# micropilot/myosuite-mjx

Hardware: AMD Instinct MI355X
Metric: env-steps/s (whole node) myoHandPoseRandom-v0 batch 4096 (higher is better)
Workload: dtype f32

## Files before the change

### myosuite_mjx_amd/csrc/myo_host.h

```cpp
#ifndef MYO_HOST_H
#define MYO_HOST_H

#include <memory>

static int g_lanes = 64;
static thread_local std::string g_err;
static int fail(int code, const std::string& msg) { g_err = msg; return code; }
#define HIPCHK(x) do { hipError_t e_ = (x); if (e_ != hipSuccess) return fail(MYO_E_HIP, std::string(#x) + ": " + hipGetErrorString(e_)); } while (0)

struct DevPool {
  std::vector<void*> ptrs;
  DevPool() = default;
  DevPool(const DevPool&) = delete;
  DevPool& operator=(const DevPool&) = delete;
  ~DevPool() { for (void* p : ptrs) (void)hipFree(p); }
  template <class T> int alloc(T** out, size_t nbytes, bool zero = true) {
    void* p = nullptr;
    const hipError_t e = hipMalloc(&p, nbytes);
    if (e != hipSuccess) return fail(e == hipErrorOutOfMemory ? MYO_E_NOMEM : MYO_E_HIP, std::string("hipMalloc: ") + hipGetErrorString(e));
    ptrs.push_back(p);
    if (zero) HIPCHK(hipMemset(p, 0, nbytes));
    *out = (T*)p;
    return MYO_OK;
  }
// ... 101 lines not shown
  bool obj_ok = false;
  std::vector<int> geom_type0, geom_body0, geom_priority0;
  std::vector<double> geom_size0, geom_pos0, geom_friction0, body_mass_d;
};

struct myo_episode { float *run = nullptr, *last = nullptr; uint8_t* finished = nullptr; int* count = nullptr; };

struct myo_obs_terms { float *terms = nullptr, *sel = nullptr, *prop = nullptr; const int2* prog = nullptr; const float* cst = nullptr; int wt = 0, ws = 0, wp = 0; };

struct myo_batch {
  const myo_model* model = nullptr;
  DevBatch db{};
  TaskDev task{};
  int ntarget_alloc = 0, obs_alloc = 0, env_offset = 0;
  DevPool pool;
  float *d_tlo = nullptr, *d_thi = nullptr, *d_init = nullptr, *d_jlo = nullptr, *d_jhi = nullptr, *d_action = nullptr, *d_rnd = nullptr;
  float* d_initv = nullptr;
  float *d_init2 = nullptr, *d_initv2 = nullptr, *d_fatvec = nullptr;
  const char* last_kernel = "step_kernel";
  DevWalk* d_walk = nullptr;
  DevTrack* d_track = nullptr;
  float* d_metrics = nullptr;
  int track_frames = 0;
  int track_flavour = 0;
  ResetArgs *d_reset = nullptr, reset_args{};
  uint64_t reset_seed = 0;
  hipEvent_t ev0 = nullptr, ev1 = nullptr;
  uint64_t bench_step = 0;
  long long* d_stamps = nullptr;
  int* d_order = nullptr;
  int* d_sched = nullptr;
  int sched_stride = 0;
  int balance = 1;
  bool bm_on = false;
  bool bp_on = false;
  int bq_body = -1;
  bool sens_on = false;
  myo_episode episode;
  myo_obs_terms obs_terms;
  bool bq_on = false;
  bool fwd_on = false;
  void* fwd_buf[16] = {};
  bool obj_on = false;
  std::vector<int> obj_geoms, obj_bodies;
  float *d_objk = nullptr, *d_obj_draw = nullptr;
  int* d_obj_draw_k = nullptr;
  std::vector<hipEvent_t> kev;
  int kev_pending = 0;
  float last_kernel_ms = 0.f;
  ~myo_batch() {
    for (hipEvent_t e : kev) (void)hipEventDestroy(e);
    if (ev0) (void)hipEventDestroy(ev0);
    if (ev1) (void)hipEventDestroy(ev1);
  }
};

struct DevBuf { void* p; size_t width, elem; };
typedef int (*BufFamily)(const myo_batch*, int which, DevBuf*);
static int buf_out(const DevBuf& d, void** dev_ptr, size_t* pitch, size_t* width) { *dev_ptr = d.p; *pitch = *width = d.width; return MYO_OK; }
static int copy_blocking(int device, void* dst, const void* src, size_t nbytes, hipMemcpyKind kind) {
  HIPCHK(hipSetDevice(device));
  HIPCHK(hipDeviceSynchronize());
  if (nbytes) HIPCHK(hipMemcpy(dst, src, nbytes, kind));
  return MYO_OK;
}
static int copy_to_host(int device, void* host, const void* dev, size_t nbytes) { return copy_blocking(device, host, dev, nbytes, hipMemcpyDeviceToHost); }
// ... 15 lines not shown

struct RwdCols { const char* const* name; int n; };
struct ObsDims { int nq, nv, nu, na, ntip, pose_act; };
enum { OBS_SRC_ROW = 0,
       OBS_SRC_TIME = 1,
       OBS_SRC_TARGET = 2,
       OBS_SRC_QPOS = 3,
       OBS_SRC_ACT = 4,
       OBS_SRC_CONST = 5 };
struct ObsTerm { const char* name; int width, src, idx; };
struct ObsTable : std::vector<ObsTerm> { int dim = 0; };

struct TaskHooks {
  int (*configure)(myo_batch*, const myo_task_config*);
  int (*obs)(myo_batch*, hipStream_t, int obs_only, int reset_only);
  int (*post)(myo_batch*, hipStream_t, uint64_t seed, int auto_max);
  RwdCols rwd;
  void (*obs_terms)(const ObsDims&, ObsTable&);
};
static const TaskHooks* task_hooks(int task);
static int launch_step(myo_batch* b, const float* action, int actmap, int nsub, hipStream_t s, int kflags = 0);

template <class Task> static int launch_task_obs(myo_batch* b, hipStream_t s, int obs_only, int reset_only) {
  hipLaunchKernelGGL(task_obs_kernel<Task>, dim3(b->db.B), dim3(64), 0, s, b->model->dm, b->db, b->task, (const DevTrack*)b->d_track, b->reset_seed, obs_only, reset_only);
  return MYO_OK;
}
static int sync_reset_args(myo_batch* b, hipStream_t s) {
  if (!b->d_reset) { const int rc = b->pool.alloc(&b->d_reset, sizeof(ResetArgs), false); if (rc) return rc; }
  else if (!memcmp(&b->reset_args.Bt, &b->db, sizeof(DevBatch)) && !memcmp(&b->reset_args.T, &b->task, sizeof(TaskDev))) return MYO_OK;
  memcpy(&b->reset_args.Bt, &b->db, sizeof(DevBatch)); memcpy(&b->reset_args.T, &b->task, sizeof(TaskDev));
  HIPCHK(hipMemcpyAsync(b->d_reset, &b->reset_args, sizeof(ResetArgs), hipMemcpyHostToDevice, s));
  return MYO_OK;
}
template <class Task> static int launch_task_post(myo_batch* b, hipStream_t s, uint64_t seed, int auto_max) {
  const int rc = sync_reset_args(b, s);
  if (rc) return rc;
  hipLaunchKernelGGL(task_post_kernel<Task>, dim3(b->db.B), dim3(64), 0, s, b->model->dm, b->db, b->task, (const DevTrack*)b->d_track,
                     (const ResetArgs*)b->d_reset, b->model->nq, b->model->dm.qpos0, seed, b->env_offset, auto_max);
  return MYO_OK;
}

static int root_link_of_dofs(const myo_model* m, int d0, int n) {
  const int l = m->dof_link[d0];
  if (m->link_parent[l] >= 0 || m->link_dofnum[l] != n) return -1;
  for (int k = 1; k < n; k++) if (m->dof_link[d0 + k] != l) return -1;
  return l;
}

static void quat2mat_d(double* R, const double* q) {
  const double w = q[0], x = q[1], y = q[2], z = q[3];
  R[0] = w * w + x * x - y * y - z * z; R[1] = 2 * (x * y - w * z); R[2] = 2 * (x * z + w * y);
  R[3] = 2 * (x * y + w * z); R[4] = w * w - x * x + y * y - z * z; R[5] = 2 * (y * z - w * x);
  R[6] = 2 * (x * z - w * y); R[7] = 2 * (y * z + w * x); R[8] = w * w - x * x - y * y + z * z;
}

#endif
```

### myosuite_mjx_amd/csrc/myo_host_batch.h

```cpp
#ifndef MYO_HOST_BATCH_H
#define MYO_HOST_BATCH_H

static int batch_create(const myo_model* m, int B, myo_batch** out) {
  HIPCHK(hipSetDevice(m->device));
  std::unique_ptr<myo_batch> owner(new myo_batch());
  myo_batch* b = owner.get();
  DevBatch& d = b->db;
  int nv = m->dm.nv, nu = m->dm.nu, nq = m->nq, rc;
  b->model = m; d.B = B; b->ntarget_alloc = nv > 24 ? nv : 24; b->obs_alloc = 3 * nv + 4 * nu + 64;
  b->sched_stride = (B + 7) / 8 + 1;
  if (m->wave_ok) {
    const int kc = m->wave_cfg == 0 ? 8 : 20, nj = m->trk ? 4 : 3;
    d.ovf_row = 8 + nj * kc + (kc + 3) / 4 + (m->trk ? TRK_STATE : 0);
    d.ovf_rows = m->trk ? NCX2 : NCX;
  }
#define BA(ptr, n) if ((rc = b->pool.alloc(&ptr, (size_t)(n) * 4))) return rc;
  BA(d.qpos, (size_t)B * nq) BA(d.qvel, (size_t)B * nv) BA(d.act, (size_t)B * nu) BA(d.ctrl, (size_t)B * nu) BA(d.warm, (size_t)B * nv)
  BA(d.time, B) BA(d.target, (size_t)B * b->ntarget_alloc) BA(d.obs, (size_t)B * b->obs_alloc) BA(d.reward, B) BA(d.done, B)
  BA(d.solved, B) BA(d.qacc, (size_t)B * nv) BA(d.tenlen, (size_t)B * nu) BA(d.actforce, (size_t)B * nu) BA(d.sitexpos, (size_t)B * 24)
  BA(d.flags, B) BA(d.diag, (size_t)B * 8) BA(d.elapsed, B) BA(d.episode, B) BA(d.mprw, (size_t)B * 64)
  BA(b->d_tlo, b->ntarget_alloc) BA(b->d_thi, b->ntarget_alloc) BA(b->d_init, nq) BA(b->d_jlo, nv) BA(b->d_jhi, nv) BA(b->d_rnd, 4 * (size_t)nq)
  BA(b->d_action, (size_t)B * nu) BA(d.fatigue, (size_t)B * 3 * nu)
  if (m->trk) { BA(d.linkx, (size_t)B * 12 * m->dm.nl) }
  if (m->wave_ok) { BA(d.ovf, (size_t)B * d.ovf_rows * d.ovf_row) BA(d.ovf_cand, (size_t)B * NCANDX) }
// ... 227 lines not shown
  FIELD(MYO_F_ACTION, b->d_action, b->model->dm.nu),
  FIELD(MYO_F_FATIGUE, b->db.fatigue, 3 * b->model->dm.nu),
  FIELD(MYO_F_HFIELD, b->db.hfield, b->model->dw.hf.nrow * b->model->dw.hf.ncol, nullptr, "MYO_F_HFIELD: the model has no colliding height field"),
  FIELD(MYO_F_GEOMSIZE, b->db.gsize, 4, nullptr, "MYO_F_GEOMSIZE: no geom override set (myo_batch_set_geom_override)"),
  FIELD(MYO_F_LINKX, b->db.linkx, 12 * b->model->dm.nl, nullptr, "MYO_F_LINKX: this model's kernel does not export link frames"),
  FIELD(MYO_F_METRICS, b->d_metrics, 4, nullptr, "MYO_F_METRICS: the track task is not configured (myo_batch_configure_track)"),
  FIELD(MYO_F_BODYMASS, b->db.bmass, b->model->body_mass0.size(), nullptr, nullptr, &bm_override),
  FIELD(MYO_F_BODYMASS_RANGE, b->db.bmass_range, 2 * b->model->body_mass0.size(), nullptr, nullptr, &bm_override),
  FIELD(MYO_F_BODYPOS, b->db.bpos, 3, nullptr, nullptr, &bp_override),
  FIELD(MYO_F_BODYPOS_RANGE, b->db.bpos_range, 6, nullptr, nullptr, &bp_override),
  FIELD(MYO_F_BODYQUAT, b->db.bquat, 4, nullptr, nullptr, &bq_override),
  FIELD(MYO_F_BODYQUAT_RANGE, b->db.bquat_range, 6, nullptr, nullptr, &bq_override),
  FIELD(MYO_F_SENSORDATA, b->db.sens, b->db.ntouch, SENS_READ_ONLY, SENS_ABSENT),
  FIELD(MYO_F_CFRC, b->db.cfrc, 3 * (b->db.ntouch + 1), SENS_READ_ONLY, SENS_ABSENT),
};
#undef FIELD
constexpr int N_FIELDS = sizeof field_rows / sizeof field_rows[0];
constexpr bool field_rows_in_id_order(int i = 0) { return i == N_FIELDS || (field_rows[i].id == i && field_rows_in_id_order(i + 1)); }
static_assert(N_FIELDS == MYO_F_CFRC + 1 && field_rows_in_id_order(), "field_rows: one row per field id of include/myo_hip.h, in id order");

static const FieldRow* field_row(int f) { return f >= 0 && f < N_FIELDS ? &field_rows[f] : nullptr; }
static int field_info(const myo_batch* b, const FieldRow* row, DevBuf* d) {
  if (!row) return fail(MYO_E_ARG, "unknown field");
  void* p = row->ptr(b);
  if (!p && row->absent) return fail(MYO_E_ARG, row->absent);
  *d = {p, row->width(b), 4};
  return MYO_OK;
}

static int batch_field(myo_batch* b, int field, void** dev_ptr, size_t* pitch, size_t* width) {
  const FieldRow* row = field_row(field);
  DevBuf d; int rc;
  if ((row && row->ov && (rc = override_start(b, *row->ov))) || (rc = field_info(b, row, &d))) return rc;
  return buf_out(d, dev_ptr, pitch, width);
}
static int batch_read(myo_batch* b, int field, void* host, size_t nbytes) {
  const FieldRow* row = field_row(field);
  DevBuf d; int rc;
  if ((rc = field_info(b, row, &d)) || (rc = buf_check(b, d, host, nbytes, "myo_batch_read: size mismatch"))) return rc;
  if (row->ov && !(b->*row->ov->on)) return row->ov->fill_default(b, field, (float*)host, b->db.B, d.width);
  return copy_to_host(b->model->device, host, d.p, nbytes);
}
static int batch_write(myo_batch* b, int field, const void* host, size_t nbytes) {
  const FieldRow* row = field_row(field);
  DevBuf d; int rc;
  if (row && row->read_only) return fail(MYO_E_ARG, row->read_only);
  if ((rc = field_info(b, row, &d)) || (rc = buf_check(b, d, host, nbytes, "myo_batch_write: size mismatch"))) return rc;
  if (row->ov && ((rc = row->ov->validate(b, field, (const float*)host, b->db.B, d.width)) || (rc = override_start(b, *row->ov)) || (rc = field_info(b, row, &d)))) return rc;
  return copy_to_device(b->model->device, d.p, host, nbytes);
}

#endif
```

### myosuite_mjx_amd/csrc/myo_host_step.h

```cpp
#ifndef MYO_HOST_STEP_H
#define MYO_HOST_STEP_H

#define MYO_WAVE_KERNELS(X)                                                                                             \
  X(WK_HAND, "step_kernel_w<24,8,32,1,3,false,0,false>", 24, 8, 32, 1, 3, false, 0)                                      \
  X(WK_HAND_SPEC, "step_kernel_w<24,8,32,1,4,false,1,false>", 24, 8, 32, 1, 4, false, 1)                                 \
  X(WK_LEG, "step_kernel_w<36,20,32,2,2,false,0,false>", 36, 20, 32, 2, 2, false, 0)                                     \
  X(WK_LEG_SCHED, "step_kernel_w<36,20,32,2,2,true,0,false>", 36, 20, 32, 2, 2, true, 0)                                 \
  X(WK_LEG_SPEC_SCHED, "step_kernel_w<36,20,32,2,2,true,2,false>", 36, 20, 32, 2, 2, true, 2)                            \
  X(WK_LEG_SPEC, "step_kernel_w<36,20,32,2,2,false,2,false>", 36, 20, 32, 2, 2, false, 2)                                \
  X(WK_TERRAIN, "step_kernel_w<36,20,32,2,2,false,0,true>", 36, 20, 32, 2, 2, false, 0, true)                            \
  X(WK_TERRAIN_SPEC_SCHED, "step_kernel_w<36,20,32,2,2,true,3,true>", 36, 20, 32, 2, 2, true, 3, true)                   \
  X(WK_TERRAIN_SPEC, "step_kernel_w<36,20,32,2,2,false,3,true>", 36, 20, 32, 2, 2, false, 3, true)                       \
  X(WK_TRK, "step_kernel_w<36,20,32,2,2,false,0,false,true>", 36, 20, 32, 2, 2, false, 0, false, true)                   \
  X(WK_HAND_RK4, "step_kernel_w<24,8,32,1,3,false,0,false,false,true>", 24, 8, 32, 1, 3, false, 0, false, false, true)   \
  X(WK_LEG_RK4, "step_kernel_w<36,20,32,2,2,false,0,false,false,true>", 36, 20, 32, 2, 2, false, 0, false, false, true)
struct WaveKernel {
  const char* name;
  void (*fn)(const DevModel*, const DevModelW*, DevBatch, const float*, int, int, long long*, const int*, const DevWalk*, int, SchedDev);
};
enum WaveKernelId {
#define X(id, name, ...) id,
  MYO_WAVE_KERNELS(X)
#undef X
  WK_TRK_OBJ
// ... 14 lines not shown
  if (m->dw.hf.on) return m->terrain_sizes ? WK_TERRAIN_SPEC : WK_TERRAIN;
  return leg_sizes ? WK_LEG_SPEC : WK_LEG;
}

static int launch_reset(myo_batch* b, const uint8_t* mask_dev, uint64_t seed, void* stream, int max_episode_steps) {
  b->reset_seed = seed;
  const DevModel& dm = b->model->dm;
  HIPCHK(hipSetDevice(b->model->device));
  hipLaunchKernelGGL(reset_kernel, dim3(b->db.B), dim3(64), 0, (hipStream_t)stream, b->db, b->task, b->model->nq, dm.nv, dm.nu, dm.qpos0, mask_dev, seed,
                     b->env_offset, max_episode_steps);
  HIPCHK(hipGetLastError());
  return MYO_OK;
}

struct SchedPlan { bool on; int grid; SchedDev S; };
static SchedPlan sched_plan(const myo_batch* b, int nsub, bool walk, int kflags) {
  const myo_model* m = b->model;
  const int Bn = b->db.B, nsubtot = nsub + (walk ? 1 : 0);
  static const int sched_mode = [] { const char* e = getenv("MYO_SCHED"); return e ? atoi(e) : -1; }();
  const int n_cu = m->n_cu > 0 ? m->n_cu : 256;
  const int resident = n_cu * (m->wave_cfg == 0 ? 16 : (m->wave_cfg == 1 ? 8 : std::max(1, (160 * 1024) / std::max(1, m->env_lds_bytes_w))));
  const bool sched_ok = !kflags && Bn >= 64 && Bn <= SCHED_ENV_MASK && nsubtot <= 15 && nsub > 0;
  const bool on = sched_ok && !b->bm_on && m->wave_cfg == 1 && !m->rk4 && !(m->dw.hf.on && !m->terrain_sizes) && (sched_mode == 1 || (sched_mode == -1 && Bn >= 2 * resident));
  const int nqueue = std::max(1, std::min(8, n_cu / 32));
  SchedPlan P{on, Bn, SchedDev{b->d_sched, b->d_sched + 32, nqueue == 8 ? b->sched_stride : (Bn + nqueue - 1) / nqueue + 1, nsubtot, nqueue}};
  if (on) {
    P.grid = Bn < resident ? Bn : resident;
    static const int grid_override = [] { const char* e = getenv("MYO_SCHED_GRID"); return e ? atoi(e) : 0; }();
    if (grid_override > 0 && grid_override < P.grid) P.grid = grid_override;
  }
  return P;
}

static int launch_wave(myo_batch* b, const float* action, int actmap, int nsub, hipStream_t s, int kflags, const DevWalk* wk) {
  const myo_model* m = b->model;
  static OncePerDevice attr;
  int rc = set_lds_limit(attr, wave_kernels, 64 * 1024, m->device);
  if (rc) return rc;
  const int Bn = b->db.B;
  const SchedPlan P = sched_plan(b, nsub, wk != nullptr, kflags);
  const int* order = nullptr;
  if (b->balance && Bn >= 1024 && Bn % 4 == 0 && !kflags && !P.on) {
    static const int prio_mode = [] { const char* e = getenv("MYO_PRIO"); return e ? atoi(e) : 2; }();
    hipLaunchKernelGGL(balance_kernel, dim3(1), dim3(1024), 0, s, (const int*)b->db.diag, Bn, b->d_order, Bn / 4, prio_mode);
    order = b->d_order;
  }
  const WaveKernel& k = wave_kernels[select_wave_kernel(m, b->bm_on, P.on, b->obj_on)];
  if (!kflags) b->last_kernel = k.name;
  if (P.on) hipLaunchKernelGGL(sched_init_kernel, dim3(1), dim3(1024), 0, s, (const int*)b->db.diag, Bn, P.S);
  hipLaunchKernelGGL(k.fn, dim3(P.grid), dim3(64), (size_t)m->env_lds_bytes_w, s, (const DevModel*)m->d_dm, (const DevModelW*)m->d_dw, b->db, action, actmap,
                     nsub, b->d_stamps, order, wk, kflags, P.S);
  HIPCHK(hipGetLastError());
  if (wk && b->db.rwd && !(kflags & KF_OBS_ONLY)) { if ((rc = walk_terms_launch(b, s))) return rc; }
  if (wk && b->obs_terms.terms) return obs_terms_launch(b, s);
  return MYO_OK;
}

static int launch_lanes(myo_batch* b, int G, const float* action, int actmap, int nsub, hipStream_t s) {
  const myo_model* m = b->model;
  const int EPW = 64 / G, grid = (b->db.B + EPW - 1) / EPW;
  const size_t lds = (size_t)EPW * m->env_lds_bytes;
  if (G == 16) hipLaunchKernelGGL(step_kernel<16>, dim3(grid), dim3(64), lds, s, m->dm, b->db, action, actmap, nsub, b->d_stamps);
  else if (G == 32) hipLaunchKernelGGL(step_kernel<32>, dim3(grid), dim3(64), lds, s, m->dm, b->db, action, actmap, nsub, b->d_stamps);
  else hipLaunchKernelGGL(step_kernel<64>, dim3(grid), dim3(64), lds, s, m->dm, b->db, action, actmap, nsub, b->d_stamps);
  HIPCHK(hipGetLastError());
  return MYO_OK;
}

static int launch_step(myo_batch* b, const float* action, int actmap, int nsub, hipStream_t s, int kflags) {
  const myo_model* m = b->model;
  const DevWalk* wk = b->task.task == MYO_TASK_WALK ? b->d_walk : nullptr;
  if (kflags && !(wk && g_lanes == 64)) return fail(MYO_E_ARG, "observation pass: walk task on the wave kernel only");
  const int G = (g_lanes == 64 && !m->wave_ok) ? 16 : ((g_lanes != 64 && !m->generic_ok) ? 64 : g_lanes);
  const bool wave = G == 64 && m->wave_ok;
  static OncePerDevice attr;
  static const struct { const void* fn; } lanes_kernels[] = {{(const void*)step_kernel<16>}, {(const void*)step_kernel<32>}, {(const void*)step_kernel<64>}, {(const void*)reach_obs_kernel<16>}};
  int rc = set_lds_limit(attr, lanes_kernels, 160 * 1024, m->device);
  if (rc) return rc;
#if MYO_POISON
  {
    static const int pmode = [] { const char* e = getenv("MYO_POISON_MODE"); return e ? atoi(e) : 7; }();
    if (pmode & 1) hipLaunchKernelGGL(scratch_poison_kernel, dim3(16384), dim3(64), 0, s, (float*)b->d_stamps, 0);
    if (pmode & 2) hipLaunchKernelGGL(vgpr_poison_kernel, dim3(8192), dim3(64), 0, s, 0x7fc0dead);
    if (pmode & 4) hipLaunchKernelGGL(sgpr_poison_kernel, dim3(32768), dim3(64), 0, s);
  }
#endif
  if (!wave && !m->generic_ok)
    return fail(MYO_E_UNSUPPORTED, "this model (tendon limits / free joint / equalities / plane contacts) needs the wave-per-env kernel (lanes = 64)");
  if (b->sens_on && (rc = sens_check(b))) return rc;
  if (b->bm_on) {
    if ((rc = bm_check(b))) return rc;
    const int n = b->db.B * m->dm.nl;
    hipLaunchKernelGGL(link_compose_kernel, dim3((n + 255) / 256), dim3(256), 0, s, b->db, m->dm.nl, m->d_lm_adr, m->d_lm_body, m->d_lm_tab);
  }
  if ((rc = obj_compose(b, s))) return rc;
  return wave ? launch_wave(b, action, actmap, nsub, s, kflags, wk) : launch_lanes(b, G, action, actmap, nsub, s);
}

static int sum_kernel_ms(myo_batch* b, int n) {
  float tot = 0.f;
  for (int i = 0; i < n; i++) { float t; HIPCHK(hipEventElapsedTime(&t, b->kev[2 * i], b->kev[2 * i + 1])); tot += t; }
  b->last_kernel_ms = tot;
  return MYO_OK;
}

int myo_bench_rollout(myo_batch* b, int steps, int nsubsteps, uint64_t seed, int mode, int max_episode_steps, void* stream, float* ms_out) {
  if (!b || steps <= 0) return fail(MYO_E_ARG, "myo_bench_rollout: bad arguments");
  HIPCHK(hipSetDevice(b->model->device));
  hipStream_t s = (hipStream_t)stream;
  int rc;
  if (!(mode & MYO_BENCH_FRESH_ACTIONS)) { rc = myo_random_action(b, b->d_action, seed, b->bench_step, b->env_offset, stream); if (rc) return rc; }
  const int base = ms_out ? 0 : b->kev_pending;
  while ((int)b->kev.size() < 2 * (base + steps)) { hipEvent_t e; HIPCHK(hipEventCreate(&e)); b->kev.push_back(e); }
  if (ms_out) { b->kev_pending = 0; HIPCHK(hipEventRecord(b->ev0, s)); }
  for (int i = 0; i < steps; i++) {
    if (mode & MYO_BENCH_FRESH_ACTIONS) { rc = myo_random_action(b, b->d_action, seed, b->bench_step++, b->env_offset, stream); if (rc) return rc; }
    HIPCHK(hipEventRecord(b->kev[2 * (base + i)], s));
    const bool mjx_track = b->task.task == MYO_TASK_TRACK && b->track_flavour == 0;
    rc = launch_step(b, b->d_action, mjx_track ? MYO_ACTMAP_CTRLRANGE : MYO_ACTMAP_MUSCLE_SIGMOID, nsubsteps, s);
    if (rc) return rc;
    HIPCHK(hipEventRecord(b->kev[2 * (base + i) + 1], s));
    const TaskHooks* hooks = task_hooks(b->task.task);
    if (mjx_track) continue;
    if ((mode & MYO_BENCH_OBS) && (mode & MYO_BENCH_AUTORESET) && max_episode_steps > 0 && hooks && hooks->post) {
      if ((rc = hooks->post(b, s, seed, max_episode_steps))) return rc;
      HIPCHK(hipGetLastError());
      continue;
    }
    if ((mode & MYO_BENCH_OBS) && b->task.task != MYO_TASK_NONE && b->task.task != MYO_TASK_WALK) { rc = launch_obs(b, s); if (rc) return rc; }
    if ((mode & MYO_BENCH_AUTORESET) && max_episode_steps > 0) {
      rc = myo_autoreset(b, max_episode_steps, seed, stream); if (rc) return rc;
      if ((mode & MYO_BENCH_OBS) && b->task.task != MYO_TASK_NONE) { rc = launch_obs(b, s, 1, 1); if (rc) return rc; }
    }
  }
  if (!ms_out) { b->kev_pending = base + steps; return MYO_OK; }
  HIPCHK(hipEventRecord(b->ev1, s));
  HIPCHK(hipEventSynchronize(b->ev1));
  HIPCHK(hipEventElapsedTime(ms_out, b->ev0, b->ev1));
  return sum_kernel_ms(b, steps);
}

const char* myo_bench_last_kernel_name(const myo_batch* b) { return b ? b->last_kernel : ""; }

int myo_bench_last_kernel_ms(myo_batch* b, float* ms_out) {
  if (!b || !ms_out) return fail(MYO_E_ARG, "null");
  if (b->kev_pending > 0) {
    HIPCHK(hipSetDevice(b->model->device));
    HIPCHK(hipEventSynchronize(b->kev[2 * b->kev_pending - 1]));
    if (const int rc = sum_kernel_ms(b, b->kev_pending)) return rc;
    b->kev_pending = 0;
  }
  *ms_out = b->last_kernel_ms;
  return MYO_OK;
}

int myo_probe_valu(int device, int waves_per_simd, int iters, double* wave_insts_per_s, int* n_cu_out) {
  if (!wave_insts_per_s || !(waves_per_simd >= 1 && waves_per_simd <= 4 || waves_per_simd == 8) || iters < 1) return fail(MYO_E_ARG, "myo_probe_valu: waves_per_simd must be 1..4 or 8");
  HIPCHK(hipSetDevice(device));
// ... 26 lines not shown
```

### myosuite_mjx_amd/csrc/myo_kernels_aux.h

```cpp
#ifndef MYO_KERNELS_AUX_H
#define MYO_KERNELS_AUX_H

__global__ void __launch_bounds__(1024) balance_kernel(const int* __restrict__ diag, int B, int* __restrict__ order, int nslot, int prio_mode) {
  __shared__ int hist[256], start[256];
  __shared__ int cmax_s;
  const int t = threadIdx.x;
  if (t < 256) hist[t] = 0;
  if (t == 0) cmax_s = 1;
  __syncthreads();
  int c4[4] = {0, 0, 0, 0};
  int cm = 1;
#pragma unroll
  for (int k = 0; k < 4; k++) { const int e = t + 1024 * k; if (e < B) { c4[k] = diag[(size_t)e * 8 + 3]; cm = max(cm, c4[k]); } }
  for (int e = t + 4096; e < B; e += 1024) cm = max(cm, diag[(size_t)e * 8 + 3]);
  for (int off = 32; off > 0; off >>= 1) cm = max(cm, __shfl_xor(cm, off));
  if ((t & 63) == 0) atomicMax(&cmax_s, cm);
  __syncthreads();
  const float sc = 255.0f / (float)cmax_s;
#define BUCKET(c) (255 - min(255, (int)(sc * (float)(c))))
#pragma unroll
  for (int k = 0; k < 4; k++) if (t + 1024 * k < B) atomicAdd(&hist[BUCKET(c4[k])], 1);
  for (int e = t + 4096; e < B; e += 1024) atomicAdd(&hist[BUCKET(diag[(size_t)e * 8 + 3])], 1);
  __syncthreads();
  if (t < 64) {
    const int h0 = hist[4 * t], h1 = hist[4 * t + 1], h2 = hist[4 * t + 2], h3 = hist[4 * t + 3];
    int tot = h0 + h1 + h2 + h3, inc = tot;
    for (int off = 1; off < 64; off <<= 1) { const int v = __shfl_up(inc, off); if (t >= off) inc += v; }
    const int base = inc - tot;
    start[4 * t] = base; start[4 * t + 1] = base + h0; start[4 * t + 2] = base + h0 + h1; start[4 * t + 3] = base + h0 + h1 + h2;
  }
  __syncthreads();
  auto place = [&](int e, int c) {
    const int r = atomicAdd(&start[BUCKET(c)], 1);
    const int q = r / nslot, i = r - q * nslot;
    const int wg = q * nslot + ((q & 1) ? nslot - 1 - i : i);
    const int pr = prio_mode == 2 ? (q < 3 ? 3 - q : 0) : (prio_mode == 1 ? (q == 0 ? 1 : 0) : (prio_mode == 3 ? (q < 2 ? 1 : 0) : 0));
    order[wg < B ? wg : r] = e | (pr << 28);
  };
#pragma unroll
  for (int k = 0; k < 4; k++) if (t + 1024 * k < B) place(t + 1024 * k, c4[k]);
  for (int e = t + 4096; e < B; e += 1024) place(e, diag[(size_t)e * 8 + 3]);
#undef BUCKET
}

__global__ void random_action_kernel(float* action, int B, int nu, uint64_t seed, uint64_t step, int env_offset) {
  size_t i = (size_t)blockIdx.x * blockDim.x + threadIdx.x;
  if (i >= (size_t)B * nu) return;
  size_t e = i / nu, k = i % nu;
  action[i] = 2.0f * u01(seed, (uint64_t)(e + env_offset) * 1024 + k, step) - 1.0f;
}

#define POL_ENVS 8
#define POL_MAXW 64
struct PolicyDev {
  int obs_dim, act_dim, nlayers;
  int width[8];
  const float* W[8];
  const float* b[8];
  const float *mean, *std;
};
__device__ __forceinline__ const float* policy_forward(const PolicyDev& P, const float* __restrict__ obs, int B, float* sh, const int j, const int le, const int e) {
  int stride = max(P.obs_dim, POL_MAXW);
  for (int l = 0; l < P.nlayers; l++) stride = max(stride, P.width[l]);
  float* xin = sh + le * stride;
  float* xout = sh + (POL_ENVS + le) * stride;
  if (e < B)
    for (int i = j; i < P.obs_dim; i += POL_MAXW) xin[i] = (obs[(size_t)e * P.obs_dim + i] - P.mean[i]) / P.std[i];
  __syncthreads();
  int nin = P.obs_dim;
  for (int l = 0; l < P.nlayers; l++) {
    const int nout = P.width[l];
    if (e < B) {
      const float* Wl = P.W[l];
      for (int jj = j; jj < nout; jj += POL_MAXW) {
        float acc = P.b[l][jj];
        for (int i = 0; i < nin; i++) acc += xin[i] * Wl[(size_t)i * nout + jj];
        xout[jj] = (l + 1 < P.nlayers) ? acc / (1.0f + expf(-acc)) : acc;
      }
    }
    __syncthreads();
    float* t = xin; xin = xout; xout = t;
    nin = nout;
// ... 175 lines not shown
}

template <void (*Body)(const DevModel&, const DevBatch&, const TaskDev&, int, int, int)>
struct StateObs {
  static __device__ __forceinline__ void obs(const DevModel& M, const DevBatch& Bt, const TaskDev& T, const DevTrack*, uint64_t, int obs_only, int e, int lane) {
    Body(M, Bt, T, obs_only, e, lane);
  }
};
template <void (*Body)(const DevModel&, const DevBatch&, const TaskDev&, const DevTrack&, uint64_t, int, int, int)>
struct TrackObs {
  static __device__ __forceinline__ void obs(const DevModel& M, const DevBatch& Bt, const TaskDev& T, const DevTrack* K, uint64_t seed, int obs_only, int e, int lane) {
    Body(M, Bt, T, *K, seed, obs_only, e, lane);
  }
};
template <class Task>
__global__ void __launch_bounds__(64) task_obs_kernel(DevModel M, DevBatch Bt, TaskDev T, const DevTrack* K, uint64_t seed, int obs_only, int reset_only) {
  const int e = blockIdx.x;
  if (e >= Bt.B) return;
  if (reset_only && Bt.elapsed[e] != 0) return;
  Task::obs(M, Bt, T, K, seed, obs_only, e, threadIdx.x);
}
template <class Task>
__global__ void __launch_bounds__(64) task_post_kernel(DevModel M, DevBatch Bt, TaskDev T, const DevTrack* K, const ResetArgs* __restrict__ R, int nq,
                                                       const float* qpos0, uint64_t seed, int env_offset, int auto_max) {
  const int e = blockIdx.x, lane = threadIdx.x;
  if (e >= Bt.B) return;
  Task::obs(M, Bt, T, K, seed, 0, e, lane);
  __syncthreads();
  if (!(Bt.done[e] > 0.f || Bt.elapsed[e] >= auto_max)) return;
  reset_body<false>(R->Bt, R->T, nq, M.nv, M.nu, qpos0, nullptr, seed, env_offset, auto_max, e, lane);
  __syncthreads();
  Task::obs(M, Bt, T, K, seed, 1, e, lane);
}

#if MYO_POISON
__global__ void __launch_bounds__(64) scratch_poison_kernel(float* sink, int n) {
  volatile float buf[512];
  for (int i = 0; i < 512; i++) buf[i] = __int_as_float(0x7fc00000 | i);
  if (n < 0) sink[threadIdx.x] = buf[(-n) & 511];
}
#define MYO_R1(p, n) p #n
#define MYO_R10(M, p, t) M(p, t##0) M(p, t##1) M(p, t##2) M(p, t##3) M(p, t##4) M(p, t##5) M(p, t##6) M(p, t##7) M(p, t##8) M(p, t##9)
#define MYO_R100(M, p, h) MYO_R10(M, p, h##0) MYO_R10(M, p, h##1) MYO_R10(M, p, h##2) MYO_R10(M, p, h##3) MYO_R10(M, p, h##4) \
                          MYO_R10(M, p, h##5) MYO_R10(M, p, h##6) MYO_R10(M, p, h##7) MYO_R10(M, p, h##8) MYO_R10(M, p, h##9)
#define MYO_R256(M, p) MYO_R10(M, p, ) MYO_R10(M, p, 1) MYO_R10(M, p, 2) MYO_R10(M, p, 3) MYO_R10(M, p, 4) MYO_R10(M, p, 5) MYO_R10(M, p, 6) \
                       MYO_R10(M, p, 7) MYO_R10(M, p, 8) MYO_R10(M, p, 9) MYO_R100(M, p, 1) MYO_R10(M, p, 20) MYO_R10(M, p, 21) MYO_R10(M, p, 22) \
                       MYO_R10(M, p, 23) MYO_R10(M, p, 24) M(p, 250) M(p, 251) M(p, 252) M(p, 253) M(p, 254) M(p, 255)
#define MYO_R102(M, p) MYO_R10(M, p, ) MYO_R10(M, p, 1) MYO_R10(M, p, 2) MYO_R10(M, p, 3) MYO_R10(M, p, 4) MYO_R10(M, p, 5) MYO_R10(M, p, 6) \
                       MYO_R10(M, p, 7) MYO_R10(M, p, 8) MYO_R10(M, p, 9) M(p, 100) M(p, 101)
#define MYO_WV(p, n) "v_mov_b32 v" #n ", %0\n\t"
#define MYO_WA(p, n) "v_accvgpr_write_b32 a" #n ", %0\n\t"
#define MYO_WS(p, n) "s_mov_b32 s" #n ", 0x7fc0beef\n\t"
#define MYO_CL(p, n) , p #n
__global__ void __launch_bounds__(64, 1) vgpr_poison_kernel(int bits) {
  asm volatile(MYO_R256(MYO_WV, "") MYO_R256(MYO_WA, "") "s_nop 0" : : "s"(bits) : "memory" MYO_R256(MYO_CL, "v") MYO_R256(MYO_CL, "a"));
}
__global__ void __launch_bounds__(64, 8) sgpr_poison_kernel() {
  asm volatile(MYO_R102(MYO_WS, "") "s_nop 0" : : : "memory" MYO_R102(MYO_CL, "s"));
}
#endif
__global__ void __launch_bounds__(1024) valu_probe_kernel(float* out, int iters, float seed) {
  extern __shared__ float lds_dummy[];
  float a0 = seed, a1 = seed + 1.f, a2 = seed + 2.f, a3 = seed + 3.f, a4 = seed + 4.f, a5 = seed + 5.f, a6 = seed + 6.f, a7 = seed + 7.f;
  const float m = 1.0000001f, c = 1e-9f * (float)threadIdx.x;
  for (int it = 0; it < iters; it++) {
#pragma unroll
// ... 11 lines not shown
```

### myosuite_mjx_amd/csrc/myo_task_myodm.h

```cpp
#ifndef MYO_TASK_MYODM_H
#define MYO_TASK_MYODM_H

__device__ __forceinline__ void myodm_obs_body(const DevModel& M, const DevBatch& Bt, const TaskDev& T, const DevTrack& K, uint64_t seed, int obs_only,
                                               const int e, const int lane) {
  const int nv = M.nv, nr = K.robot_dim;
  const int vdim = K.has_vel ? nr : 1, oe = 2 * nv + nr + vdim;
  const auto [o, q, v, a, dt] = task_row(M, Bt, T, e, nv);
  const int elapsed = Bt.elapsed[e];
  track_lookup<true>(K, e, e + Bt.env_offset, 0.f, elapsed, lane, (double)elapsed * (double)T.frame_skip * (double)M.timestep,
                     seed + 0x632BE59BD9B4E019ull * (uint64_t)Bt.episode[e]);
  __syncthreads();
  const float* R = K.ref + (size_t)e * K.ref_pitch;
  const float* tc = R + 2 * nr;
  float p[3] = {0.f, 0.f, 0.f}, Rb[9], x[2][3];
  if (lane < 2) link_chain<true>(M, Bt, q, e, lane == 0 ? K.obj_link : K.wrist_link, lane == 0 ? K.obj_p : K.wrist_p, K.obj_R, p, Rb);
  site_gather<2>(M, Bt, e, lane, 0, p, x);
  const float *com = x[0], *wr = x[1];
  for (int i = lane; i < nv; i += 64) { o[i] = q[i]; o[nv + i] = v[i]; }
  float qe = 0.f, ve = 0.f;
  if (lane < nr) {
    qe = q[lane] - R[lane];
    o[2 * nv + lane] = qe;
    if (K.has_vel) { ve = v[lane] - R[nr + lane]; o[2 * nv + nr + lane] = ve; }
  }
// ... 68 lines not shown
  if ((rc = pool.upload(&K.T, c->ref_time, (size_t)c->horizon)) || (rc = pool.upload(&K.robot, c->ref_robot, nrobot)) ||
      (K.has_vel && (rc = pool.upload(&K.robot_vel, c->ref_robot_vel, nrobot))) ||
      (rc = pool.upload(&K.object, c->ref_object, (size_t)c->object_horizon * c->object_dim)) || (rc = pool.upload(&K.init_qpos, c->init_qpos, (size_t)nq)) ||
      (rc = pool.upload(&K.lo, c->ctrl_lo, (size_t)nu)) || (rc = pool.upload(&K.hi, c->ctrl_hi, (size_t)nu))) return rc;
  K.obj_link = c->object_link; K.wrist_link = c->wrist_link;
  for (int k = 0; k < 3; k++) { K.obj_p[k] = c->object_ipos[k]; K.wrist_p[k] = c->wrist_ipos[k]; }
  for (int k = 0; k < 9; k++) K.obj_R[k] = c->object_imat[k];
  K.lift_z = c->lift_z; K.obj_err_scale = c->obj_err_scale; K.base_err_scale = c->base_err_scale; K.lift_bonus_mag = c->lift_bonus_mag;
  K.qpos_w = c->qpos_reward_weight; K.qpos_err_scale = c->qpos_err_scale; K.qvel_w = c->qvel_reward_weight; K.qvel_err_scale = c->qvel_err_scale;
  K.obj_fail2 = c->obj_fail_thresh * c->obj_fail_thresh; K.base_fail2 = c->base_fail_thresh * c->base_fail_thresh; K.qpos_fail = c->qpos_fail_thresh;
  K.w_pose = c->w_pose; K.w_object = c->w_object; K.w_bonus = c->w_bonus; K.w_penalty = c->w_penalty;
  K.ref_pitch = 2 * c->robot_dim + c->object_dim;
  K.seed = c->seed;
  if ((rc = pool.alloc(&K.ref, (size_t)B * K.ref_pitch * 4)) || (!b->d_metrics && (rc = pool.alloc(&b->d_metrics, (size_t)B * 4 * 4))) ||
      (!b->d_track && (rc = pool.alloc(&b->d_track, sizeof(DevTrack))))) return rc;
  K.metrics = b->d_metrics;
  HIPCHK(hipMemcpy(b->d_track, &K, sizeof(DevTrack), hipMemcpyHostToDevice));
  b->db.track = b->d_track;
  b->track_frames = c->n_frames;
  b->track_flavour = c->flavour;
  TaskDev& T = b->task;
  T = TaskDev{};
  T.task = MYO_TASK_TRACK; T.frame_skip = c->n_frames; T.nq = nq; T.obs_dim = obs_dim;
  HIPCHK(hipMemcpy(b->d_init, c->init_qpos, (size_t)nq * 4, hipMemcpyHostToDevice));
  T.init_qpos = b->d_init; T.jnt_lo = b->d_jlo; T.jnt_hi = b->d_jhi; T.target_lo = b->d_tlo; T.target_hi = b->d_thi;
  return MYO_OK;
}

static int track_obs(myo_batch* b, hipStream_t s, int obs_only, int reset_only) {
  return b->track_flavour == 1 ? launch_task_obs<MyodmTask>(b, s, obs_only, reset_only) : launch_task_obs<MjxTrackTask>(b, s, obs_only, reset_only);
}
static int track_post(myo_batch* b, hipStream_t s, uint64_t seed, int max_episode_steps) {
  b->reset_seed = seed;
  return launch_task_post<MyodmTask>(b, s, seed, max_episode_steps);
}
static const TaskHooks track_hooks = {nullptr, track_obs, track_post};

#endif
```

Baseline: 4.554 million.

## Fuse next-step random actions and placement into post-step interstep kernel

Adds an interstep kernel that replaces the task post kernel in the benchmark loop. It also generates the next step's random actions inside the same launch and can optionally compute the balance placement order in extra high-priority blocks. Action generation is then skipped when the same actions are already known, which saves a separate random_action launch (and optionally the balance launch) per step. The cost is more state tracking on the host for action validity and order freshness, and the balance kernel is generalised through a templated deal helper.

```diff
diff --git a/myosuite_mjx_amd/csrc/myo_host.h b/myosuite_mjx_amd/csrc/myo_host.h
--- a/myosuite_mjx_amd/csrc/myo_host.h
+++ b/myosuite_mjx_amd/csrc/myo_host.h
@@ -157,6 +157,12 @@
   int* d_sched = nullptr;
   int sched_stride = 0;
   int balance = 1;
+  bool order_fresh = false;
+  bool action_known = false;
+  bool action_shared = false;
+  uint64_t action_seed = 0, action_step = 0;
+  int action_offset = 0;
+  struct { bool on = false, actions = false, place = false; uint64_t step = 0; } inter;
   bool bm_on = false;
   bool bp_on = false;
   int bq_body = -1;
@@ -238,9 +244,22 @@
   HIPCHK(hipMemcpyAsync(b->d_reset, &b->reset_args, sizeof(ResetArgs), hipMemcpyHostToDevice, s));
   return MYO_OK;
 }
-template <class Task> static int launch_task_post(myo_batch* b, hipStream_t s, uint64_t seed, int auto_max) {
+static int placement_prio() { static const int v = [] { const char* e = getenv("MYO_PRIO"); return e ? atoi(e) : 2; }(); return v; }
+static int placement_deal_mode() { static const int v = [] { const char* e = getenv("MYO_DEAL"); return e && atoi(e) == 1 ? 1 : 0; }(); return v; }
+template <class Task> static int launch_interstep(myo_batch* b, hipStream_t s, uint64_t seed, int auto_max) {
+  const int Bn = b->db.B;
+  const bool place = b->inter.place && Bn <= 64 * INTERSTEP_CAP && Bn % 4 == 0;
+  const InterstepNext N{b->inter.actions ? b->d_action : nullptr, b->inter.step, place ? b->d_order : nullptr, Bn / 4, placement_prio(), placement_deal_mode()};
+  hipLaunchKernelGGL(interstep_kernel<Task>, dim3(Bn + (place ? INTERSTEP_NP : 0)), dim3(64), 0, s, b->model->dm, b->db, b->task, (const DevTrack*)b->d_track,
+                     (const ResetArgs*)b->d_reset, b->model->nq, b->model->dm.qpos0, seed, b->env_offset, auto_max, N);
+  b->order_fresh = place;
+  if (b->inter.actions) { b->action_known = true; b->action_seed = seed; b->action_step = b->inter.step; b->action_offset = b->env_offset; }
+  return MYO_OK;
+}
+template <class Task, bool INTER = true> static int launch_task_post(myo_batch* b, hipStream_t s, uint64_t seed, int auto_max) {
   const int rc = sync_reset_args(b, s);
   if (rc) return rc;
+  if constexpr (INTER) { if (b->inter.on) return launch_interstep<Task>(b, s, seed, auto_max); }
   hipLaunchKernelGGL(task_post_kernel<Task>, dim3(b->db.B), dim3(64), 0, s, b->model->dm, b->db, b->task, (const DevTrack*)b->d_track,
                      (const ResetArgs*)b->d_reset, b->model->nq, b->model->dm.qpos0, seed, b->env_offset, auto_max);
   return MYO_OK;
diff --git a/myosuite_mjx_amd/csrc/myo_host_batch.h b/myosuite_mjx_amd/csrc/myo_host_batch.h
--- a/myosuite_mjx_amd/csrc/myo_host_batch.h
+++ b/myosuite_mjx_amd/csrc/myo_host_batch.h
@@ -283,6 +283,7 @@
   const FieldRow* row = field_row(field);
   DevBuf d; int rc;
   if ((row && row->ov && (rc = override_start(b, *row->ov))) || (rc = field_info(b, row, &d))) return rc;
+  if (field == MYO_F_ACTION) { b->action_shared = true; b->action_known = false; }
   return buf_out(d, dev_ptr, pitch, width);
 }
 static int batch_read(myo_batch* b, int field, void* host, size_t nbytes) {
@@ -298,6 +299,7 @@
   if (row && row->read_only) return fail(MYO_E_ARG, row->read_only);
   if ((rc = field_info(b, row, &d)) || (rc = buf_check(b, d, host, nbytes, "myo_batch_write: size mismatch"))) return rc;
   if (row->ov && ((rc = row->ov->validate(b, field, (const float*)host, b->db.B, d.width)) || (rc = override_start(b, *row->ov)) || (rc = field_info(b, row, &d)))) return rc;
+  if (field == MYO_F_ACTION) b->action_known = false;
   return copy_to_device(b->model->device, d.p, host, nbytes);
 }
 
diff --git a/myosuite_mjx_amd/csrc/myo_host_step.h b/myosuite_mjx_amd/csrc/myo_host_step.h
--- a/myosuite_mjx_amd/csrc/myo_host_step.h
+++ b/myosuite_mjx_amd/csrc/myo_host_step.h
@@ -70,6 +70,12 @@
   return P;
 }
 
+static int step_lanes(const myo_model* m) { return (g_lanes == 64 && !m->wave_ok) ? 16 : ((g_lanes != 64 && !m->generic_ok) ? 64 : g_lanes); }
+static bool placement_wanted(const myo_batch* b, bool sched_on) {
+  const int Bn = b->db.B;
+  return b->balance && Bn >= 1024 && Bn % 4 == 0 && Bn <= 1024 * BALANCE_CAP && !sched_on;
+}
+
 static int launch_wave(myo_batch* b, const float* action, int actmap, int nsub, hipStream_t s, int kflags, const DevWalk* wk) {
   const myo_model* m = b->model;
   static OncePerDevice attr;
@@ -78,11 +84,11 @@
   const int Bn = b->db.B;
   const SchedPlan P = sched_plan(b, nsub, wk != nullptr, kflags);
   const int* order = nullptr;
-  if (b->balance && Bn >= 1024 && Bn % 4 == 0 && !kflags && !P.on) {
-    static const int prio_mode = [] { const char* e = getenv("MYO_PRIO"); return e ? atoi(e) : 2; }();
-    hipLaunchKernelGGL(balance_kernel, dim3(1), dim3(1024), 0, s, (const int*)b->db.diag, Bn, b->d_order, Bn / 4, prio_mode);
+  if (placement_wanted(b, P.on) && !kflags) {
+    if (!b->order_fresh) hipLaunchKernelGGL(balance_kernel, dim3(1), dim3(1024), 0, s, (const int*)b->db.diag, Bn, b->d_order, Bn / 4, placement_prio(), placement_deal_mode());
     order = b->d_order;
   }
+  b->order_fresh = false;
   const WaveKernel& k = wave_kernels[select_wave_kernel(m, b->bm_on, P.on, b->obj_on)];
   if (!kflags) b->last_kernel = k.name;
   if (P.on) hipLaunchKernelGGL(sched_init_kernel, dim3(1), dim3(1024), 0, s, (const int*)b->db.diag, Bn, P.S);
@@ -109,8 +115,9 @@
   const myo_model* m = b->model;
   const DevWalk* wk = b->task.task == MYO_TASK_WALK ? b->d_walk : nullptr;
   if (kflags && !(wk && g_lanes == 64)) return fail(MYO_E_ARG, "observation pass: walk task on the wave kernel only");
-  const int G = (g_lanes == 64 && !m->wave_ok) ? 16 : ((g_lanes != 64 && !m->generic_ok) ? 64 : g_lanes);
+  const int G = step_lanes(m);
   const bool wave = G == 64 && m->wave_ok;
+  if (!wave) b->order_fresh = false;
   static OncePerDevice attr;
   static const struct { const void* fn; } lanes_kernels[] = {{(const void*)step_kernel<16>}, {(const void*)step_kernel<32>}, {(const void*)step_kernel<64>}, {(const void*)reach_obs_kernel<16>}};
   int rc = set_lds_limit(attr, lanes_kernels, 160 * 1024, m->device);
@@ -147,12 +154,22 @@
   HIPCHK(hipSetDevice(b->model->device));
   hipStream_t s = (hipStream_t)stream;
   int rc;
-  if (!(mode & MYO_BENCH_FRESH_ACTIONS)) { rc = myo_random_action(b, b->d_action, seed, b->bench_step, b->env_offset, stream); if (rc) return rc; }
+  static const bool interstep = [] { const char* e = getenv("MYO_INTERSTEP"); return !e || atoi(e) != 0; }();
+  static const bool interstep_place = [] { const char* e = getenv("MYO_INTERSTEP_PLACE"); return e && atoi(e) != 0; }();
+  const bool fresh = (mode & MYO_BENCH_FRESH_ACTIONS) != 0;
+  if (b->action_shared) b->action_known = false;
+  auto actions = [&](uint64_t step) -> int {
+    if (fresh && b->action_known && b->action_seed == seed && b->action_step == step && b->action_offset == b->env_offset) return MYO_OK;
+    const int r = myo_random_action(b, b->d_action, seed, step, b->env_offset, stream);
+    b->action_known = !r; b->action_seed = seed; b->action_step = step; b->action_offset = b->env_offset;
+    return r;
+  };
+  if (!fresh && (rc = actions(b->bench_step))) return rc;
   const int base = ms_out ? 0 : b->kev_pending;
   while ((int)b->kev.size() < 2 * (base + steps)) { hipEvent_t e; HIPCHK(hipEventCreate(&e)); b->kev.push_back(e); }
   if (ms_out) { b->kev_pending = 0; HIPCHK(hipEventRecord(b->ev0, s)); }
   for (int i = 0; i < steps; i++) {
-    if (mode & MYO_BENCH_FRESH_ACTIONS) { rc = myo_random_action(b, b->d_action, seed, b->bench_step++, b->env_offset, stream); if (rc) return rc; }
+    if (fresh) { if ((rc = actions(b->bench_step))) return rc; b->bench_step++; }
     HIPCHK(hipEventRecord(b->kev[2 * (base + i)], s));
     const bool mjx_track = b->task.task == MYO_TASK_TRACK && b->track_flavour == 0;
     rc = launch_step(b, b->d_action, mjx_track ? MYO_ACTMAP_CTRLRANGE : MYO_ACTMAP_MUSCLE_SIGMOID, nsubsteps, s);
@@ -161,7 +178,13 @@
     const TaskHooks* hooks = task_hooks(b->task.task);
     if (mjx_track) continue;
     if ((mode & MYO_BENCH_OBS) && (mode & MYO_BENCH_AUTORESET) && max_episode_steps > 0 && hooks && hooks->post) {
-      if ((rc = hooks->post(b, s, seed, max_episode_steps))) return rc;
+      if (interstep) {
+        b->inter.on = true; b->inter.actions = fresh; b->inter.step = b->bench_step;
+        b->inter.place = interstep_place && step_lanes(b->model) == 64 && b->model->wave_ok && placement_wanted(b, sched_plan(b, nsubsteps, false, 0).on);
+      }
+      rc = hooks->post(b, s, seed, max_episode_steps);
+      b->inter.on = false;
+      if (rc) return rc;
       HIPCHK(hipGetLastError());
       continue;
     }
diff --git a/myosuite_mjx_amd/csrc/myo_kernels_aux.h b/myosuite_mjx_amd/csrc/myo_kernels_aux.h
--- a/myosuite_mjx_amd/csrc/myo_kernels_aux.h
+++ b/myosuite_mjx_amd/csrc/myo_kernels_aux.h
@@ -1,26 +1,41 @@
 #ifndef MYO_KERNELS_AUX_H
 #define MYO_KERNELS_AUX_H
 
-__global__ void __launch_bounds__(1024) balance_kernel(const int* __restrict__ diag, int B, int* __restrict__ order, int nslot, int prio_mode) {
-  __shared__ int hist[256], start[256];
+#include <type_traits>
+
+template <int G, int CAP, int NT, class F>
+__device__ __forceinline__ void for_own_envs(int B, F&& f) {
+  if constexpr (G < CAP) {
+    if (NT * G < B) {
+      f(std::integral_constant<int, G>{}); f(std::integral_constant<int, G + 1>{}); f(std::integral_constant<int, G + 2>{}); f(std::integral_constant<int, G + 3>{});
+      for_own_envs<G + 4, CAP, NT>(B, f);
+    }
+  }
+}
+template <int NT, int CAP, int NP = 1>
+__device__ __forceinline__ void placement_deal(const int* __restrict__ diag, int B, int* __restrict__ order, int nslot, int prio_mode, int deal, const int t, const int p = 0) {
+  __shared__ int hist[256], start[256], lower[NP > 1 ? 256 : 1];
   __shared__ int cmax_s;
-  const int t = threadIdx.x;
-  if (t < 256) hist[t] = 0;
+  for (int i = t; i < 256; i += NT) { hist[i] = 0; if (NP > 1) lower[i] = 0; }
   if (t == 0) cmax_s = 1;
   __syncthreads();
-  int c4[4] = {0, 0, 0, 0};
+  int c[CAP];
   int cm = 1;
-#pragma unroll
-  for (int k = 0; k < 4; k++) { const int e = t + 1024 * k; if (e < B) { c4[k] = diag[(size_t)e * 8 + 3]; cm = max(cm, c4[k]); } }
-  for (int e = t + 4096; e < B; e += 1024) cm = max(cm, diag[(size_t)e * 8 + 3]);
+  const int n = t < B ? (B - 1 - t) / NT + 1 : 0;
+#define FOR_OWN_ENVS(k, ...) for_own_envs<0, CAP, NT>(B, [&](auto k_) __attribute__((always_inline)) { constexpr int k = decltype(k_)::value; __VA_ARGS__ })
+  FOR_OWN_ENVS(k, c[k] = k < n ? diag[((size_t)t + (size_t)k * NT) * 8 + 3] : 0;);
+  FOR_OWN_ENVS(k, cm = max(cm, c[k]););
   for (int off = 32; off > 0; off >>= 1) cm = max(cm, __shfl_xor(cm, off));
   if ((t & 63) == 0) atomicMax(&cmax_s, cm);
   __syncthreads();
   const float sc = 255.0f / (float)cmax_s;
-#define BUCKET(c) (255 - min(255, (int)(sc * (float)(c))))
-#pragma unroll
-  for (int k = 0; k < 4; k++) if (t + 1024 * k < B) atomicAdd(&hist[BUCKET(c4[k])], 1);
-  for (int e = t + 4096; e < B; e += 1024) atomicAdd(&hist[BUCKET(diag[(size_t)e * 8 + 3])], 1);
+  FOR_OWN_ENVS(k,
+    c[k] = 255 - min(255, (int)(sc * (float)c[k]));
+    if (k < n) {
+      atomicAdd(&hist[c[k]], 1);
+      if (NP > 1 && k % NP < p) atomicAdd(&lower[c[k]], 1);
+    }
+  );
   __syncthreads();
   if (t < 64) {
     const int h0 = hist[4 * t], h1 = hist[4 * t + 1], h2 = hist[4 * t + 2], h3 = hist[4 * t + 3];
@@ -28,26 +43,33 @@
     for (int off = 1; off < 64; off <<= 1) { const int v = __shfl_up(inc, off); if (t >= off) inc += v; }
     const int base = inc - tot;
     start[4 * t] = base; start[4 * t + 1] = base + h0; start[4 * t + 2] = base + h0 + h1; start[4 * t + 3] = base + h0 + h1 + h2;
-  }
-  __syncthreads();
-  auto place = [&](int e, int c) {
-    const int r = atomicAdd(&start[BUCKET(c)], 1);
-    const int q = r / nslot, i = r - q * nslot;
-    const int wg = q * nslot + ((q & 1) ? nslot - 1 - i : i);
-    const int pr = prio_mode == 2 ? (q < 3 ? 3 - q : 0) : (prio_mode == 1 ? (q == 0 ? 1 : 0) : (prio_mode == 3 ? (q < 2 ? 1 : 0) : 0));
-    order[wg < B ? wg : r] = e | (pr << 28);
-  };
-#pragma unroll
-  for (int k = 0; k < 4; k++) if (t + 1024 * k < B) place(t + 1024 * k, c4[k]);
-  for (int e = t + 4096; e < B; e += 1024) place(e, diag[(size_t)e * 8 + 3]);
-#undef BUCKET
-}
-
+    if (NP > 1)
+      for (int j = 0; j < 4; j++) start[4 * t + j] += lower[4 * t + j];
+  }
+  __syncthreads();
+  const int prio_tab = prio_mode == 2 ? 0x0123 : (prio_mode == 1 ? 0x0001 : (prio_mode == 3 ? 0x0011 : 0));
+  FOR_OWN_ENVS(k, if (k % NP == p && k < n) c[k] = atomicAdd(&start[c[k]], 1););
+  FOR_OWN_ENVS(k,
+    if (k % NP != p || k >= n) return;
+    const int e = t + NT * k, r = c[k];
+    const int q = (r >= nslot) + (r >= 2 * nslot) + (r >= 3 * nslot), i = r - q * nslot;
+    int wg = q * nslot + ((q & 1) ? nslot - 1 - i : i);
+    if (deal == 1 && q > 0) { const int u = B - 1 - r; wg = (1 + u % 3) * nslot + u / 3; }
+    order[wg < B ? wg : r] = e | (((prio_tab >> (4 * q)) & 3) << 28);
+  );
+#undef FOR_OWN_ENVS
+}
+#define BALANCE_CAP 64
+__global__ void __launch_bounds__(1024) balance_kernel(const int* __restrict__ diag, int B, int* __restrict__ order, int nslot, int prio_mode, int deal) {
+  placement_deal<1024, BALANCE_CAP>(diag, B, order, nslot, prio_mode, deal, threadIdx.x);
+}
+
+__device__ __forceinline__ float bench_action(uint64_t seed, uint64_t ge, uint64_t k, uint64_t step) { return 2.0f * u01(seed, ge * 1024 + k, step) - 1.0f; }
 __global__ void random_action_kernel(float* action, int B, int nu, uint64_t seed, uint64_t step, int env_offset) {
   size_t i = (size_t)blockIdx.x * blockDim.x + threadIdx.x;
   if (i >= (size_t)B * nu) return;
   size_t e = i / nu, k = i % nu;
-  action[i] = 2.0f * u01(seed, (uint64_t)(e + env_offset) * 1024 + k, step) - 1.0f;
+  action[i] = bench_action(seed, (uint64_t)(e + env_offset), k, step);
 }
 
 #define POL_ENVS 8
@@ -289,6 +311,29 @@
   __syncthreads();
   Task::obs(M, Bt, T, K, seed, 1, e, lane);
 }
+#define INTERSTEP_CAP 64
+#define INTERSTEP_NP 4
+struct InterstepNext { float* action; uint64_t step; int* order; int nslot, prio_mode, deal; };
+template <class Task>
+__global__ void __launch_bounds__(64) interstep_kernel(DevModel M, DevBatch Bt, TaskDev T, const DevTrack* K, const ResetArgs* __restrict__ R, int nq,
+                                                       const float* qpos0, uint64_t seed, int env_offset, int auto_max, InterstepNext N) {
+  const int lane = threadIdx.x;
+  if (N.order && blockIdx.x < INTERSTEP_NP) {
+    __builtin_amdgcn_s_setprio(3);
+    placement_deal<64, INTERSTEP_CAP, INTERSTEP_NP>(Bt.diag, Bt.B, N.order, N.nslot, N.prio_mode, N.deal, lane, blockIdx.x);
+    return;
+  }
+  const int e = (int)blockIdx.x - (N.order ? INTERSTEP_NP : 0);
+  if (e >= Bt.B) return;
+  if (N.action)
+    for (int k = lane; k < M.nu; k += 64) N.action[(size_t)e * M.nu + k] = bench_action(seed, (uint64_t)(e + env_offset), k, N.step);
+  Task::obs(M, Bt, T, K, seed, 0, e, lane);
+  __syncthreads();
+  if (!(Bt.done[e] > 0.f || Bt.elapsed[e] >= auto_max)) return;
+  reset_body<false>(R->Bt, R->T, nq, M.nv, M.nu, qpos0, nullptr, seed, env_offset, auto_max, e, lane);
+  __syncthreads();
+  Task::obs(M, Bt, T, K, seed, 1, e, lane);
+}
 
 #if MYO_POISON
 __global__ void __launch_bounds__(64) scratch_poison_kernel(float* sink, int n) {
diff --git a/myosuite_mjx_amd/csrc/myo_task_myodm.h b/myosuite_mjx_amd/csrc/myo_task_myodm.h
--- a/myosuite_mjx_amd/csrc/myo_task_myodm.h
+++ b/myosuite_mjx_amd/csrc/myo_task_myodm.h
@@ -124,7 +124,7 @@
 }
 static int track_post(myo_batch* b, hipStream_t s, uint64_t seed, int max_episode_steps) {
   b->reset_seed = seed;
-  return launch_task_post<MyodmTask>(b, s, seed, max_episode_steps);
+  return launch_task_post<MyodmTask, false>(b, s, seed, max_episode_steps);
 }
 static const TaskHooks track_hooks = {nullptr, track_obs, track_post};
 
```

Measured after the change: 4.556 million (median of 2 runs). About the same (+0.0%).
